# DataArcTech/RAG-ARC

Measured on AMD Instinct MI355X. Metric: queries/sec at fixed (N_corpus, d), exact top-k (ids bit-exact vs CPU oracle), higher is better.
Workload: dtype f16; 1 GPU; 100000000x768 fp16 corpus of N(0,1) directions resident in HBM, row-sharded over 1 GPU(s), batch 256 queries, cosine top-100, exact (canonical fp32 rescore); n_corpus=100000000, d=768, batch=256, k=100, rows_per_gpu=100000000, exchange=none (one shard), repaired_queries_last_step=0

## Files before the change

include/rarc.h:

```cpp
#ifndef RARC_H
#define RARC_H

#include <stddef.h>
#include <stdint.h>

#ifdef __cplusplus
extern "C" {
#endif

#define RARC_VERSION 600

#define RARC_OK 0
#define RARC_E_INVALID -1
#define RARC_E_HIP -2
#define RARC_E_WORKSPACE -3
#define RARC_E_UNSUPPORTED -4
#define RARC_E_IO -5

#define RARC_MAX_QUERIES 256
#define RARC_MAX_K 1024
#define RARC_DIM_ALIGN 128

#define RARC_Q_OK 0u
#define RARC_Q_UNCERTAIN 1u
// ... 261 lines not shown
int rarc_file_to_device(const char* path, int n_seg, const int64_t* h_file_off, const int64_t* h_bytes,
                        const int64_t* h_dev_off, void* d_base, int64_t d_capacity_bytes, void* h_staging,
                        size_t staging_bytes, int n_threads, int flags, void* stream, RarcIoStats* stats);
int rarc_device_to_file(const char* path, int n_seg, const int64_t* h_file_off, const int64_t* h_bytes,
                        const int64_t* h_dev_off, const void* d_base, int64_t d_capacity_bytes, void* h_staging,
                        size_t staging_bytes, int n_threads, int flags, void* stream, RarcIoStats* stats);

size_t rarc_wide_workspace_bytes(int d_pad, int cand_cap);
int rarc_search_wide(const void* d_rows, const uint16_t* d_image16, int fmt, int64_t n_rows, int d_pad, float max_norm,
                     float rho, const void* d_qblock, int nq, int k, int64_t id_base, int64_t* d_out_ids,
                     float* d_out_scores, uint32_t* d_status, void* d_ws, size_t ws_bytes, int cand_cap, void* stream);

int rarc_row_sqnorms(const void* d_rows, int fmt, int64_t n_rows, int d_pad, int64_t first_row, float* d_xn, void* stream);
int rarc_search_wide_l2(const void* d_rows, const uint16_t* d_image16, int fmt, int64_t n_rows, int d_pad, float max_norm,
                        float rho, const float* d_xn, const void* d_qblock, int nq, int k, int64_t id_base, int64_t* d_out_ids,
                        float* d_out_scores, uint32_t* d_status, void* d_ws, size_t ws_bytes, int cand_cap, void* stream);
int rarc_debug_wide_bounds(const void* d_ws, size_t ws_bytes, int d_pad, int cand_cap, float* d_out, void* stream);
int rarc_debug_query_scale8(float mx, float* sq, float* qi);
int rarc_debug_q8_tail_plan(uint32_t t_begin, uint32_t n_tiles, uint32_t grid, int d_pad, int fmt, int pct, int min_mib,
                            uint32_t* t_dyn, uint32_t* r0, uint32_t* unit);
int rarc_debug_q8_tail_chunks(uint32_t k_first, uint32_t n, uint32_t stride, uint32_t unit, uint32_t t_dyn, uint32_t r0,
                              uint32_t n_tiles, uint32_t* t0, uint32_t* t_end);
int64_t rarc_debug_q8_tail_counter_offset(int launch);

size_t rarc_search_rows_workspace_bytes(int nq, int k);
int rarc_search_rows(const void* d_rows, int fmt, int64_t n_rows, int d_pad, const void* d_qblock, int nq, const int64_t* d_list,
                     int64_t m, int k, int64_t id_base, const float* d_xn, int l2, int64_t* d_out_ids, float* d_out_scores,
                     uint32_t* d_status, void* d_ws, size_t ws_bytes, void* stream);
int rarc_strike_rows(const int64_t* d_ids, const float* d_scores, int nq, int kprime, const uint32_t* d_bits, int64_t n_rows,
                     int64_t id_base, int k, int l2, int64_t* d_out_ids, float* d_out_scores, uint32_t* d_count, void* stream);

size_t rarc_search_rows_grouped_workspace_bytes(int nq, int k);
int rarc_search_rows_grouped(const void* d_rows, int fmt, int64_t n_rows, int d_pad, const void* d_qblock, int nq,
                             const int64_t* d_lists, const int64_t* d_tiles, int n_tiles, int64_t m_max, int k, int64_t id_base,
                             const float* d_xn, int l2, int64_t* d_out_ids, float* d_out_scores, uint32_t* d_status, void* d_ws,
                             size_t ws_bytes, void* stream);
int rarc_strike_rows_grouped(const int64_t* d_ids, const float* d_scores, int nq, int kprime, const uint32_t* d_bits,
                             const int64_t* d_bits_off, int64_t n_rows, int64_t id_base, int k, int l2, int64_t* d_out_ids,
                             float* d_out_scores, uint32_t* d_count, void* stream);

size_t rarc_similar_pairs_workspace_bytes(int64_t n_rows, int d, int cand_cap);
int rarc_similar_pairs(const float* d_rows, int64_t ld, int64_t n_rows, int d, double threshold, void* d_ws, size_t ws_bytes,
                       int cand_cap, int64_t* d_out_pairs, double* d_out_scores, int64_t out_cap,
                       unsigned long long* d_out_count, uint32_t* d_flags, void* stream);

size_t rarc_knn_graph_workspace_bytes(int64_t n_rows, int d, int top_k, int cand_cap);
// ... 156 lines not shown
```

rag-arc_amd/csrc/scan_q8.hip:

```cpp
#include "rarc_common.h"
#include <stdio.h>
#ifdef RARC_Q8_ABLATIONS
#include <algorithm>
#endif

struct ScanQ8Params {
  const uint4* corpus;
  const float* tmeta;
  const float* hq;
  const int8_t* q8;
  const float* qinv;
  const float* eps8;
  uint32_t n_rows;
  uint32_t n_tiles;
  uint32_t t_begin;
  uint32_t resume;
  float hot_margin;
  uint32_t* thr;
  const float* binlo;
  const float* binscale;
  const float* bininv;
  uint32_t* hist;
  uint32_t* cnt2;
  uint64_t* cand;
  uint32_t seg;
  uint32_t kprime;
  uint32_t nq;
  uint32_t t_dyn;
  uint32_t tail_r0;
  uint32_t* tail_ctr;
  unsigned long long* dbg;
};

#ifndef Q8_M16_FP16_ROWS
#define Q8_M16_FP16_ROWS 0
#endif
#ifndef Q8_BIG_PF
#define Q8_BIG_PF 1
#endif
#ifndef Q8_BIG_NG
#define Q8_BIG_NG 2
#endif
#ifndef Q8_EB
#define Q8_EB 0
#endif
constexpr int Q8_WAVES = 8;
constexpr int Q8_THREADS = Q8_WAVES * 64;

constexpr int Q8_WSTAGE = 768;
constexpr int Q8_STAGE = 8 * Q8_WSTAGE;
constexpr int Q8_TB_SLOTS = 16;
constexpr int Q8_TB_STRIDE = 80;
constexpr int Q8_DBG_BYTES = 65536;
constexpr int Q8_FIN_SLOT = 2048;
// ... 50 lines not shown
  const uint64_t first = (uint64_t)t_dyn + (uint64_t)start * stride + slot, end = (uint64_t)t_dyn + (uint64_t)(start + r) * stride;
  *t0 = first < n_tiles ? (uint32_t)first : n_tiles;
  *t_end = end < n_tiles ? (uint32_t)end : n_tiles;
}

inline bool q8_tail_plan(uint32_t t_begin, uint32_t n_tiles, uint32_t g, uint32_t unit, uint32_t pct, uint64_t tile_bytes,
                         uint64_t min_bytes, uint32_t* t_dyn, uint32_t* r0) {
  *t_dyn = n_tiles;
  *r0 = 0;
  if (g == 0 || unit == 0 || n_tiles <= t_begin) return false;
  const uint32_t rounds = (uint32_t)(((uint64_t)(n_tiles - t_begin) + g - 1) / g);
  const uint32_t share = (uint32_t)((uint64_t)rounds * (pct > 100u ? 100u : pct) / 100u);
  if (share < unit || (uint64_t)rounds * tile_bytes < min_bytes) return false;
  uint32_t stat = (rounds - share) / unit * unit;
  if (stat < unit) stat = unit;
  const uint64_t td = (uint64_t)t_begin + (uint64_t)stat * g;
  if (td >= n_tiles) return false;
  *t_dyn = (uint32_t)td;
  *r0 = (uint32_t)((((uint64_t)(n_tiles - *t_dyn) + g - 1) / g / 2) / unit * unit);
  return true;
}
inline uint32_t q8_tail_unit(int d_pad) { return d_pad <= 384 ? 4u : 2u; }

template <int D, int FMT = 0, int ABL = 0>
__global__ __launch_bounds__(Q8_THREADS) void rarc_scan_q8_kernel(const ScanQ8Params p) {
  static_assert(D % 128 == 0 && D >= 128 && D <= 1024, "D must be a multiple of 128, <= 1024");
  extern __shared__ __attribute__((aligned(16))) char smem[];
  using L = ScanQ8Lds<D, (FMT != 0) || Q8_M16_FP16_ROWS>;
  constexpr int KS = D / 32;
  static_assert(FMT == 0 || D % 256 == 0, "fp8 rows are padded to a multiple of 256");
  constexpr int EPC = FMT ? 16 : 8;
  constexpr int CPR = D / EPC;
  constexpr int CPT = 32 * CPR / Q8_THREADS;
  constexpr int MSTRIDE = FMT == 1 ? RARC_QMETA_F8_STRIDE : RARC_QMETA_STRIDE;
  constexpr int TCH = 32 * CPR;
  constexpr bool NT_ROWS = !(ABL & 262144);

  const int tid = threadIdx.x;
  const int wave = __builtin_amdgcn_readfirstlane(tid >> 6);
  const int lane = tid & 63;
  const int row = lane & 31, h = lane >> 5;
  constexpr bool M16 = (FMT != 0) || Q8_M16_FP16_ROWS;
  const uint32_t q_lo = wave * 32 + (lane & 15);
  const uint32_t qidx = M16 ? q_lo + 16 * (lane >> 5) : wave * 32 + row;
  const int rq = lane >> 4;
  const int rql = rq & 1;
// ... 23 lines not shown
  if constexpr (M16) {
    const int8_t* qp = p.q8 + (size_t)q_lo * D + 16 * rq;
#pragma unroll
    for (int ks = 0; ks < KS2; ++ks) {
      qf[2 * ks] = *(const i32x4*)(qp + 64 * ks);
      qf[2 * ks + 1] = *(const i32x4*)(qp + 16 * D + 64 * ks);
    }
  } else {
    const int8_t* qp = p.q8 + (size_t)qidx * D + 16 * h;
#pragma unroll
    for (int ks = 0; ks < KS; ++ks) qf[ks] = *(const i32x4*)(qp + 32 * ks);
  }
  const float my_qinv = p.qinv[qidx];
  const float my_hq = p.hq[qidx];
  const float r_max = p.tmeta[0 - RARC_QMETA_HDR];
  float thr = __uint_as_float(p.thr[qidx]);
  __builtin_amdgcn_s_waitcnt(0x0F70);

  constexpr bool WOFF_REGS = (D <= 768);
  auto woff_of = [&](int j) {
    const uint32_t c = j * Q8_THREADS + tid;
    return (c / CPR) * L::RS + (c % CPR) * EPC;
  };
  uint32_t woff[WOFF_REGS ? CPT : 1];
  if constexpr (WOFF_REGS) {
#pragma unroll
    for (int j = 0; j < CPT; ++j) woff[j] = woff_of(j);
  }
  const uint32_t aoff = M16 ? (lane & 15) * L::RS + 16 * rq : row * L::RS + 16 * h;

  const uint32_t stride = gridDim.x;
  uint32_t t0 = p.t_begin + blockIdx.x, t_end = p.tail_ctr ? p.t_dyn : p.n_tiles;
  const bool has_own = blockIdx.x < p.nq;
  const uint32_t own_q = has_own ? blockIdx.x : 0u;
  const uint32_t* hword = p.hist + (size_t)own_q * RARC_NB + 32 * wave + row;

  struct Fetch {
    uint4 c[CPT];
    float mul[FMT == 1 ? CPT : 1];
    float2 meta;
    uint32_t thr;
    uint32_t hw;
  };
  auto clamp_tile = [&](uint32_t t) { return t < t_end ? t : 0u; };
  auto fetch = [&](Fetch& f, uint32_t tile, auto refresh) {
    if constexpr (ABL & 524288) f.meta = make_float2(__uint_as_float(0x7c003c00u), 1.0f);
    else f.meta = *(const float2*)(p.tmeta + (size_t)tile * MSTRIDE);
    if constexpr (FMT == 1) {
#pragma unroll
      for (int j = 0; j < CPT; ++j)
        f.mul[j] = p.tmeta[(size_t)tile * MSTRIDE + 2 + (j * Q8_THREADS + tid) / CPR];
    }
    if constexpr (decltype(refresh)::value) {
      f.thr = __hip_atomic_load(&p.thr[qidx], __ATOMIC_RELAXED, __HIP_MEMORY_SCOPE_AGENT);
      f.hw = __hip_atomic_load(hword, __ATOMIC_RELAXED, __HIP_MEMORY_SCOPE_AGENT);
    }
    __builtin_amdgcn_sched_barrier(0);
    const uint4* src = p.corpus + (size_t)tile * TCH + tid;
#pragma unroll
    for (int j = 0; j < CPT; ++j) {
      if constexpr (NT_ROWS)
        f.c[j] = __builtin_bit_cast(uint4, __builtin_nontemporal_load((const q8_u32x4*)(src + j * Q8_THREADS)));
      else
        f.c[j] = src[j * Q8_THREADS];
    }
  };
  uint32_t opaque_zero = 0;
  asm volatile("" : "+v"(opaque_zero));
  auto convert_chunk = [&](const Fetch& f, int j, half_t s, char* dst) {
    char* at = dst + (WOFF_REGS ? woff[WOFF_REGS ? j : 0] : woff_of(j));
    if constexpr (FMT == 2) {
      const uint4 v = f.c[j];
      *(uint4*)at = make_uint4(v.x ^ opaque_zero, v.y ^ opaque_zero, v.z ^ opaque_zero, v.w ^ opaque_zero);
    } else if constexpr (FMT == 1) {
      if (ABL & 16) {
        const uint4 v = f.c[j];
        *(uint4*)at = make_uint4(v.x ^ opaque_zero, v.y ^ opaque_zero, v.z ^ opaque_zero, v.w ^ opaque_zero);
      } else {
        const uint4 v = rarc_quant8_chunk_f8(f.c[j], (half_t)f.mul[j]);
        if (ABL & 32768) asm volatile("" ::"v"(v.x), "v"(v.y), "v"(v.z), "v"(v.w));
        else *(uint4*)at = v;
      }
    } else {
      uint2 o;
      if (ABL & 16) { o.x = f.c[j].x ^ f.c[j].z; o.y = f.c[j].y ^ f.c[j].w; }
      else o = rarc_quant8_chunk(f.c[j], s);
      *(uint2*)at = o;
    }
  };
  auto convert_tile = [&](const Fetch& f, int buf) {
    const half_t s = q8_tile_scale(f.meta.x);
    char* dst = smem + buf * L::TILE;
#pragma unroll
// ... 10 lines not shown
      constexpr int CSTEP = KS2 / CPT;
      i32x4 a0[PF], a1[PF];
      if (!(ABL & 4) && !((ABL & 65536) && wave >= 4)) {
#pragma unroll
        for (int i = 0; i < PF; ++i) {
          a0[i] = *(const i32x4*)(a_base + 64 * i);
          a1[i] = *(const i32x4*)(a_base + 16 * L::RS + 64 * i);
        }
      }
#pragma unroll
      for (int ks = 0; ks < KS2; ++ks) {
        if (!(ABL & 4) && !((ABL & 65536) && wave >= 4)) {
          c00 = __builtin_amdgcn_mfma_i32_16x16x64_i8(a0[ks % PF], qf[2 * ks], c00, 0, 0, 0);
          c01 = __builtin_amdgcn_mfma_i32_16x16x64_i8(a0[ks % PF], qf[2 * ks + 1], c01, 0, 0, 0);
          c10 = __builtin_amdgcn_mfma_i32_16x16x64_i8(a1[ks % PF], qf[2 * ks], c10, 0, 0, 0);
          c11 = __builtin_amdgcn_mfma_i32_16x16x64_i8(a1[ks % PF], qf[2 * ks + 1], c11, 0, 0, 0);
          if (ks + PF < KS2 && !(ABL & 131072)) {
            a0[ks % PF] = *(const i32x4*)(a_base + 64 * (ks + PF));
            a1[ks % PF] = *(const i32x4*)(a_base + 16 * L::RS + 64 * (ks + PF));
          }
        }
        if (ks % CSTEP == CSTEP / 2) convert_chunk(nx, ks / CSTEP, s, dst);
      }
      if constexpr (D <= 512 || D > 768) RARC_MFMA_SETTLE(c11);
      return (i32x16){c00[0], c00[1], c00[2], c00[3], c10[0], c10[1], c10[2], c10[3],
                      c01[0], c01[1], c01[2], c01[3], c11[0], c11[1], c11[2], c11[3]};
    } else {
      i32x16 c0 = {0};
      constexpr int PF = (D <= 768) ? 4 : 2;
      constexpr int CSTEP = KS / CPT;
      i32x4 a[PF];
      if (!(ABL & 4)) {
#pragma unroll
        for (int i = 0; i < PF; ++i) a[i] = *(const i32x4*)(a_base + 32 * i);
      }
#pragma unroll
      for (int ks = 0; ks < KS; ++ks) {
        if (!(ABL & 4)) {
          c0 = __builtin_amdgcn_mfma_i32_32x32x32_i8(a[ks % PF], qf[ks], c0, 0, 0, 0);
          if (ks + PF < KS) a[ks % PF] = *(const i32x4*)(a_base + 32 * (ks + PF));
        }
        if (ks % CSTEP == CSTEP / 2) convert_chunk(nx, ks / CSTEP, s, dst);
      }
      if constexpr (D <= 512) RARC_MFMA_SETTLE(c0);
      return c0;
    }
  };
  auto regroup = [&](i32x16& a) __attribute__((always_inline)) {
    asm volatile("v_nop\n\tv_nop\n\t"
                 "v_permlane32_swap_b32 %0, %8\n\tv_permlane32_swap_b32 %1, %9\n\tv_permlane32_swap_b32 %2, %10\n\t"
                 "v_permlane32_swap_b32 %3, %11\n\tv_permlane32_swap_b32 %4, %12\n\tv_permlane32_swap_b32 %5, %13\n\t"
                 "v_permlane32_swap_b32 %6, %14\n\tv_permlane32_swap_b32 %7, %15"
                 : "+v"(a[0]), "+v"(a[1]), "+v"(a[2]), "+v"(a[3]), "+v"(a[4]), "+v"(a[5]), "+v"(a[6]), "+v"(a[7]),
                   "+v"(a[8]), "+v"(a[9]), "+v"(a[10]), "+v"(a[11]), "+v"(a[12]), "+v"(a[13]), "+v"(a[14]), "+v"(a[15]));
  };

  auto emit = [&](uint32_t q, uint64_t key, bool hot) {
    const uint32_t slot = atomicAdd(&s_cnt[q], 1u);
    if (slot < p.seg) p.cand[((size_t)q * RARC_MAX_WG + blockIdx.x) * p.seg + slot] = key;
    if (hot) atomicAdd(&p.hist[q * RARC_NB + rarc_bin_of(rarc_candscore(key), s_binlo[q], s_binscale[q])], 1u);
  };
  uint32_t wcount = 0;
  uint64_t* my_skey = s_skey + wave * Q8_WSTAGE;
  uint8_t* my_sq = s_sq + wave * Q8_WSTAGE;
  auto stage_q = [&](bool want, float a, uint32_t doc, uint32_t qq) __attribute__((always_inline)) {
    const unsigned long long b = __builtin_amdgcn_ballot_w64(want);
    if (b == 0) return;
// ... 142 lines not shown
    fetch(f[1], clamp_tile(t0 + stride), Q8Flag<true>{});
    __builtin_amdgcn_sched_barrier(0);
    fetch(f[2], clamp_tile(t0 + 2 * stride), Q8Flag<true>{});
    __builtin_amdgcn_sched_barrier(0);
    fetch(f[3], clamp_tile(t0 + 3 * stride), Q8Flag<true>{});
    __builtin_amdgcn_sched_barrier(0);
    if (!grp_b) fetch(f[0], clamp_tile(t0 + 4 * stride), Q8Flag<true>{});
  } else if constexpr (NG == 2) {
    fetch(f[1], clamp_tile(t0 + stride), Q8Flag<true>{});
    __builtin_amdgcn_sched_barrier(0);
    if (!grp_b) fetch(f[0], clamp_tile(t0 + 2 * stride), Q8Flag<true>{});
  } else {
    fetch(f[0], clamp_tile(t0 + stride), Q8Flag<true>{});
  }
  __builtin_amdgcn_sched_barrier(0);
  __builtin_amdgcn_s_waitcnt(0x0F70);
  q8_lds_barrier();

  i32x16 acc_b = {0};
  bool live_prev = false;
#define Q8_STAMP(slot)                                                                                        \
  if ((ABL & 1024) && blockIdx.x == 0 && it >= 1000 && it < 1016 && lane == 0)                                 \
    p.dbg[8 + ((it - 1000) * Q8_WAVES + wave) * 8 + (slot)] = __builtin_amdgcn_s_memtime();
#define Q8_RF_FETCH(g, par) (!(ABL & 8) && (NG == 1 ? (par) == 1 : (g) == 1))
#define Q8_RF_USE(g, par) (!(ABL & 8) && (NG == 1 ? (par) == 0 : (g) == 1))
#define Q8_ITER(PAR, GB, G, GP)                                                                               \
  {                                                                                                           \
    Q8_STAMP(0)                                                                                               \
    if (!(GB)) {             \
      const float tinv = mcur[PAR].y, tsc = mcur[PAR].x;                                                      \
      i32x16 acc;                                                                                             \
      acc = mfma_convert(PAR, f[G]);                                                                  \
      mcur[(PAR) ^ 1] = f[G].meta;                                                                    \
      Q8_STAMP(1)                                                                                             \
      if (Q8_RF_USE(G, PAR)) {                                                                                \
        thr = fmaxf(thr, __uint_as_float(f[G].thr));                                                  \
        if (lane < 32) s_hland[32 * wave + lane] = f[G].hw;                                           \
      }                                                                                                       \
      if constexpr (EB) {                                \
        Q8_STAMP(3)                                                                                           \
        q8_lds_barrier();                                                                                     \
        Q8_STAMP(4)                                                                                           \
      }                                                                                                       \
      if (!(ABL & 1) && live) prune(acc, cur, tinv, tsc);                                                     \
      else if (q8_all16(acc) == 0x7fffffff) p.cnt2[0] = 1;  \
      Q8_STAMP(2)                                                                                             \
                                                                \
      if (!(ABL & 2)) fetch(f[G], clamp_tile(cur + (NG + 1) * stride), Q8Flag<Q8_RF_FETCH(G, PAR)>{});        \
    } else {  \
      if (!(ABL & 1) && live_prev) prune(acc_b, cur - stride, mcur[(PAR) ^ 1].y, mcur[(PAR) ^ 1].x);          \
      live_prev = live;                                                                                       \
      Q8_STAMP(1)                                                                                             \
      if (!(ABL & 2)) fetch(f[GP], clamp_tile(cur + NG * stride), Q8Flag<Q8_RF_FETCH(GP, PAR)>{});            \
      __builtin_amdgcn_sched_barrier(0);           \
      Q8_STAMP(2)                                                                                             \
      acc_b = mfma_convert(PAR, f[G]);                                                                        \
      mcur[(PAR) ^ 1] = f[G].meta;                                                                            \
      if (Q8_RF_USE(G, PAR)) {                                                                                \
        thr = fmaxf(thr, __uint_as_float(f[G].thr));                                                          \
        if (lane < 32) s_hland[32 * wave + lane] = f[G].hw;                                                   \
      }                                                                                                       \
      if ((ABL & 1) && q8_all16(acc_b) == 0x7fffffff) p.cnt2[0] = 1;                                          \
    }                                                                                                         \
    if constexpr (!EB) {                                                                                      \
      Q8_STAMP(3)                                                                                             \
      q8_lds_barrier();                                                                                       \
      Q8_STAMP(4)                                                                                             \
    }                                                                                                         \
    ++it;                                                                                                     \
                      \
    if (!(ABL & 8) && wave == 0 && has_own && (it <= 16 || (it & 3) == 0)) {                                  \
      const int b = rarc_wave_find_from_top_256(s_hland[4 * lane], s_hland[4 * lane + 1],                     \
                                                s_hland[4 * lane + 2], s_hland[4 * lane + 3], p.kprime);      \
      if (b >= 2 && lane == 0) {                                                                              \
        const float lo = s_binlo[own_q];                                                                      \
        const float t = fmaxf(rarc_bin_threshold(b, lo, s_bininv[own_q]) - 2.0002f * s_eps8[own_q], lo);      \
        if (t > last_pub) {                  \
          last_pub = t;                                                                                       \
          __hip_atomic_store(&p.thr[own_q], __float_as_uint(t), __ATOMIC_RELAXED, __HIP_MEMORY_SCOPE_AGENT);  \
        }                                                                                                     \
      }                                                                                                       \
    }                                                                                                         \
                  \
    if (!(ABL & 64) && (wcount | tb_n) != 0 &&                                                                 \
        (it <= 16 || (it & (it - 1)) == 0 || (it & 127) == 0 || wcount > (uint32_t)Q8_WSTAGE / 2))            \
      flush();                                                                                                \
  }

#define Q8_STEP(OFF, PAR, GB, G, GP)                                                  \
    {                                                                                 \
      const uint32_t cur = base + (OFF) * stride;                                     \
      const bool live = (OFF) == 0 || cur < t_end;                                \
      Q8_ITER(PAR, GB, G, GP)                                                         \
    }
#define Q8_LOOP(GB)                                                                   \
  if constexpr (NG == 4) {                                                            \
    for (uint32_t base = t0; base < t_end; base += 4 * stride) {                  \
      Q8_STEP(0, 0, GB, 1, 0) Q8_STEP(1, 1, GB, 2, 1) Q8_STEP(2, 0, GB, 3, 2) Q8_STEP(3, 1, GB, 0, 3) \
    }                                                                                 \
  } else {                                                                            \
    for (uint32_t base = t0; base < t_end; base += 2 * stride) {                  \
      Q8_STEP(0, 0, GB, NG == 2 ? 1 : 0, 0) Q8_STEP(1, 1, GB, 0, NG == 2 ? 1 : 0)     \
    }                                                                                 \
  }
  if (grp_b) {
    Q8_LOOP(true)
  } else {
    Q8_LOOP(false)
  }
#undef Q8_STEP
#undef Q8_LOOP
#undef Q8_ITER
#undef Q8_RF_FETCH
#undef Q8_RF_USE
  if (grp_b && !(ABL & 1) && live_prev)
    prune(acc_b, t0 + (((t_end - 1 - t0) / stride) | (NG == 4 ? 3u : 1u)) * stride, mcur[1].y, mcur[1].x);
  t0 = p.n_tiles;
  if (p.tail_ctr) {
    uint32_t* s_tick = (uint32_t*)(smem + L::TICK);
    if (tid == 0) *s_tick = atomicAdd(p.tail_ctr, 1u);
    __syncthreads();
    const uint32_t k = __builtin_amdgcn_readfirstlane(*s_tick);
    q8_tail_chunk(k, stride, NG == 4 ? 4u : 2u, p.t_dyn, p.tail_r0, p.n_tiles, &t0, &t_end);
  }
  } while (t0 < p.n_tiles);
  flush();
  __syncthreads();
  if (tid < RARC_MAX_QUERIES) p.cnt2[(size_t)blockIdx.x * RARC_MAX_QUERIES + tid] = s_cnt[tid];
  if (p.dbg && blockIdx.x == 0 && tid == 0) {
    p.dbg[0] = __builtin_amdgcn_s_memtime() - dbg_c0;
    p.dbg[1] = __builtin_amdgcn_s_memrealtime() - dbg_r0;
  }
#ifdef RARC_Q8_ABLATIONS
  if (!(ABL & 1024) && p.dbg && tid == 0) {
// ... 113 lines not shown
        }
        return RARC_OK;
      }
      if (abl == 512) return launch_scan_q8<D, FMT, 512>(p, grid, s);
      if (abl == 17) return launch_scan_q8<D, FMT, 17>(p, grid, s);
      if (abl == 21) return launch_scan_q8<D, FMT, 21>(p, grid, s);
      if (abl == 32769) return launch_scan_q8<D, FMT, 32769>(p, grid, s);
      if (abl == 32773) return launch_scan_q8<D, FMT, 32773>(p, grid, s);
      if (abl == 131073) return launch_scan_q8<D, FMT, 131073>(p, grid, s);
      if (abl == 65536) return launch_scan_q8<D, FMT, 65536>(p, grid, s);
      if (abl == 65537) return launch_scan_q8<D, FMT, 65537>(p, grid, s);
    }
  }
#endif
  hipEvent_t e0, e1;
  const bool prof = rarc_prof_next(&e0, &e1);
  if (prof) RARC_HIP_CHECK(hipEventRecord(e0, s));
  hipLaunchKernelGGL((rarc_scan_q8_kernel<D, FMT, ABL>), dim3(grid), dim3(Q8_THREADS), lds, s, p);
  RARC_HIP_CHECK(hipGetLastError());
  if (prof) RARC_HIP_CHECK(hipEventRecord(e1, s));
  return RARC_OK;
}

template <int FMTV>
static int dispatch_scan_q8(const ScanQ8Params& p, int d_pad, int grid, hipStream_t s) {
  switch (d_pad) {
    case 256: return launch_scan_q8<256, FMTV>(p, grid, s);
    case 512: return launch_scan_q8<512, FMTV>(p, grid, s);
    case 768: return launch_scan_q8<768, FMTV>(p, grid, s);
    case 1024: return launch_scan_q8<1024, FMTV>(p, grid, s);
    default: break;
  }
  if (FMTV == 0) {
    switch (d_pad) {
      case 128: return launch_scan_q8<128, 0>(p, grid, s);
      case 384: return launch_scan_q8<384, 0>(p, grid, s);
      case 640: return launch_scan_q8<640, 0>(p, grid, s);
      case 896: return launch_scan_q8<896, 0>(p, grid, s);
      default: break;
    }
  }
  rarc_set_error("rarc_scan_q8 (row format %d): padded dim %d unsupported (multiple of %d, <= 1024)", FMTV, d_pad,
                 FMTV == 0 ? 128 : 256);
  return RARC_E_UNSUPPORTED;
}

int rarc_scan_q8_launch(const void* corpus, const float* rowscale, int fmt, int64_t n_rows, int d_pad,
                        const float* qmeta, const uint16_t* q16, const int8_t* q8, const float* qinv,
                        const float* eps16, const float* eps8, int nq, int kprime, float bin_lo, float bin_hi,
                        const RarcWs& ws, int cap, int* grid_out, hipStream_t s, const int8_t* shadow8,
                        int (*tighten)(void* ctx, int n_wg, int mode), void* tighten_ctx, const float* hq, const float* floor,
                        int* hybrid_out) {
  ScanQ8Params p;
  p.hq = hq;
  p.corpus = fmt == 2 ? (const uint4*)shadow8 : (const uint4*)corpus;
  p.tmeta = qmeta + RARC_QMETA_HDR;
  p.q8 = q8;
  p.qinv = qinv;
  p.eps8 = eps8;
  p.n_rows = (uint32_t)n_rows;
  p.n_tiles = (uint32_t)((n_rows + 31) / 32);
  p.t_begin = 0;
  p.resume = 0;
  p.hot_margin = 1.0f;
  p.thr = (uint32_t*)ws.thr;
  p.binlo = ws.binlo;
  p.binscale = ws.binscale;
  p.bininv = ws.bininv;
  p.hist = ws.hist;
  p.cnt2 = ws.cnt2;
  p.cand = ws.cand;
  p.seg = (uint32_t)(cap / RARC_MAX_WG);
  p.kprime = (uint32_t)kprime;
  p.nq = (uint32_t)nq;
  p.dbg = nullptr;
  p.t_dyn = p.n_tiles;
  p.tail_r0 = 0;
  p.tail_ctr = nullptr;

  int dev = 0, cus = 256;
  RARC_HIP_CHECK(hipGetDevice(&dev));
  RARC_HIP_CHECK(hipDeviceGetAttribute(&cus, hipDeviceAttributeMultiprocessorCount, dev));
  int grid = cus < RARC_MAX_WG ? cus : RARC_MAX_WG;
  if (const char* e = getenv("RARC_SCAN_Q8_WGS")) { const int g = atoi(e); if (g >= 8 && g < grid) grid = g; }
  if ((uint32_t)grid > p.n_tiles) grid = (int)p.n_tiles;
  *grid_out = grid;
  auto launch = [&](const ScanQ8Params& pp) {
    return fmt == 2 ? dispatch_scan_q8<2>(pp, d_pad, grid, s)
                    : fmt == 1 ? dispatch_scan_q8<1>(pp, d_pad, grid, s) : dispatch_scan_q8<0>(pp, d_pad, grid, s);
  };
  int tail_pct = 16;
  if (const char* e = getenv("RARC_SCAN_Q8_TAIL")) tail_pct = atoi(e);
  tail_pct = tail_pct < 0 ? 0 : (tail_pct > 100 ? 100 : tail_pct);
  int tail_min_mib = 32;
  if (const char* e = getenv("RARC_SCAN_Q8_TAIL_MIN")) tail_min_mib = atoi(e);
  const uint64_t tile_bytes = 32ull * (uint64_t)d_pad * (fmt == 0 ? 2u : 1u);
  static_assert(Q8_DEEP_D == 384, "q8_tail_unit");
  auto set_tail = [&](ScanQ8Params& pp, int launch_idx) {
    const bool tail = q8_tail_plan(pp.t_begin, pp.n_tiles, (uint32_t)grid, q8_tail_unit(d_pad), (uint32_t)tail_pct, tile_bytes,
                                   (uint64_t)(tail_min_mib > 0 ? tail_min_mib : 0) << 20, &pp.t_dyn, &pp.tail_r0);
    pp.tail_ctr = tail ? ws.flags + RARC_WS_TAIL_FLAG + launch_idx : nullptr;
  };
  static const int split_mode = getenv("RARC_SCAN_SPLIT") ? atoi(getenv("RARC_SCAN_SPLIT")) : 3;
  const uint32_t pair = 2u * (uint32_t)(grid > 0 ? grid : 1);
  uint32_t cuts[3];
  int n_cuts = 0;
  if (tighten && split_mode > 0) {
    uint32_t div[3] = {512u, 64u, 8u};
    if (const char* e = getenv("RARC_SPLIT_DIVS")) {
      unsigned a = 0, b = 0, c = 0;
      const int got = sscanf(e, "%u,%u,%u", &a, &b, &c);
      if (got >= 1) { div[0] = a; div[1] = got >= 2 ? b : 0; div[2] = got >= 3 ? c : 0; }
    }
    for (int i = (split_mode >= 3 ? 0 : (split_mode == 2 ? 1 : 2)); i < 3; ++i) {
      if (div[i] == 0) continue;
      const uint32_t t = (p.n_tiles / div[i]) / pair * pair;
      static const int min_env = getenv("RARC_SPLIT_MIN") ? atoi(getenv("RARC_SPLIT_MIN")) : 0;
      const uint32_t min_pairs = min_env > 0 ? (uint32_t)min_env : (div[i] == 8u ? 16u : 8u);
      if (t >= min_pairs * pair && (n_cuts == 0 || t > cuts[n_cuts - 1])) cuts[n_cuts++] = t;
    }
  }
  int rc = rarc_seed_launch(corpus, rowscale, fmt == 2 ? 0 : fmt, n_rows, d_pad, q16, nq, kprime, bin_lo, bin_hi, eps16,
                            eps8, ws, s, n_cuts ? (int64_t)cuts[0] * 32 : 0, floor);
  if (rc) return rc;
  if (p.n_tiles == 0) return RARC_OK;
  RARC_REQUIRE(rarc_gate_scan(s) == 0, RARC_E_HIP, "rarc_scan_q8: hipStreamWaitEvent on the gate event failed");
  uint32_t begin = 0;
  static const int hybrid_env = getenv("RARC_HYBRID") ? atoi(getenv("RARC_HYBRID")) : 1;
  static const int hybrid_div = getenv("RARC_HYBRID_DIV") ? atoi(getenv("RARC_HYBRID_DIV")) : 8;
  if (hybrid_out) *hybrid_out = 0;
  if (hybrid_out && hybrid_env && tighten && fmt == 0 && d_pad <= 768 && n_cuts == 0 && hybrid_div >= 2) {
    const uint32_t stage = (p.n_tiles / (uint32_t)hybrid_div) / pair * pair;
    if (stage >= 2u * pair && stage < p.n_tiles) {
      if ((rc = rarc_scan_f16_stage_launch((const uint16_t*)corpus, n_rows, stage, d_pad, q16, eps16, nq, kprime, ws, cap, grid,
                                           s)) != RARC_OK)
        return rc;
      if ((rc = tighten(tighten_ctx, grid, 2)) != RARC_OK) return rc;
      ScanQ8Params pi = p;
      pi.t_begin = stage;
      pi.resume = 1u;
      pi.hot_margin = 0.f;
      *hybrid_out = 1;
      set_tail(pi, 0);
      return launch(pi);
    }
  }
  for (int i = 0; i <= n_cuts; ++i) {
    ScanQ8Params pi = p;
    pi.t_begin = begin;
    pi.n_tiles = i < n_cuts ? cuts[i] : p.n_tiles;
    pi.resume = i > 0 ? 1u : 0u;
    pi.hot_margin = i > 0 ? 0.f : 1.0f;
    set_tail(pi, i);
    if ((rc = launch(pi)) != RARC_OK) return rc;
    if (i < n_cuts && (rc = tighten(tighten_ctx, grid, 1)) != RARC_OK) return rc;
    begin = pi.n_tiles;
  }
  return RARC_OK;
}

extern "C" int rarc_debug_q8_tail_plan(uint32_t t_begin, uint32_t n_tiles, uint32_t grid, int d_pad, int fmt, int pct, int min_mib,
                                       uint32_t* t_dyn, uint32_t* r0, uint32_t* unit) {
  RARC_REQUIRE(t_dyn && r0 && unit, RARC_E_INVALID, "rarc_debug_q8_tail_plan: null pointer");
  RARC_REQUIRE(d_pad > 0 && fmt >= 0 && fmt <= 2, RARC_E_INVALID, "rarc_debug_q8_tail_plan: d_pad %d, row format %d", d_pad, fmt);
  *unit = q8_tail_unit(d_pad);
  q8_tail_plan(t_begin, n_tiles, grid, *unit, (uint32_t)(pct < 0 ? 0 : pct), 32ull * (uint64_t)d_pad * (fmt == 0 ? 2u : 1u),
               (uint64_t)(min_mib > 0 ? min_mib : 0) << 20, t_dyn, r0);
  return RARC_OK;
}
extern "C" int rarc_debug_q8_tail_chunks(uint32_t k_first, uint32_t n, uint32_t stride, uint32_t unit, uint32_t t_dyn, uint32_t r0,
                                         uint32_t n_tiles, uint32_t* t0, uint32_t* t_end) {
  RARC_REQUIRE(t0 && t_end && stride > 0 && unit > 0, RARC_E_INVALID, "rarc_debug_q8_tail_chunks: null pointer, stride or unit 0");
  for (uint32_t i = 0; i < n; ++i) q8_tail_chunk(k_first + i, stride, unit, t_dyn, r0, n_tiles, &t0[i], &t_end[i]);
  return RARC_OK;
}
extern "C" int64_t rarc_debug_q8_tail_counter_offset(int launch) {
  return launch >= 0 && launch < 4 ? (int64_t)(RARC_WS_FLAGS + 4 * (size_t)(RARC_WS_TAIL_FLAG + launch)) : -1;
}
```

rag-arc_amd/hip/binding.py:

```python
from __future__ import annotations

import ctypes
import os
import threading
from ctypes import c_double, c_float, c_int, c_int64, c_size_t, c_uint64, c_void_p

_PKG = os.path.dirname(os.path.dirname(os.path.abspath(__file__)))
_LIB = os.environ.get("RARC_LIBRARY") or os.path.join(_PKG, "lib", "librarc_hip.so")

MAX_QUERIES = 256
MAX_K = 1024
WIDE_MAX_K = 8192
WIDE_MAX_DPAD = 4096
DIM_ALIGN = 128
Q_UNCERTAIN = 1
Q_OVERFLOW = 2
WS_ANYFLAG_OFFSET = 5124


class RarcError(RuntimeError):
    """Raised for every non-zero status returned by librarc_hip.so."""


class RarcUnsupported(RarcError, NotImplementedError):
# ... 165 lines not shown
    "rarc_lm_gather_last": (c_int, [c_void_p, c_int, c_int, c_int, c_int, c_void_p, c_void_p]),
    "rarc_wordpiece_create": (c_int, [ctypes.c_char_p, c_size_t, c_int, ctypes.c_char_p, ctypes.c_char_p, ctypes.c_char_p,
                                      ctypes.c_char_p, ctypes.c_char_p, c_size_t, c_int, ctypes.POINTER(c_void_p)]),
    "rarc_wordpiece_destroy": (None, [c_void_p]),
    "rarc_wordpiece_encode": (c_int, [c_void_p, ctypes.c_char_p, c_void_p, c_int, c_int, c_void_p, c_int64, c_void_p, c_int]),
    "rarc_file_to_device": (c_int, [ctypes.c_char_p, c_int, ctypes.POINTER(c_int64), ctypes.POINTER(c_int64),
                                    ctypes.POINTER(c_int64), c_void_p, c_int64, c_void_p, c_size_t, c_int, c_int, c_void_p,
                                    ctypes.POINTER(IoStats)]),
    "rarc_device_to_file": (c_int, [ctypes.c_char_p, c_int, ctypes.POINTER(c_int64), ctypes.POINTER(c_int64),
                                    ctypes.POINTER(c_int64), c_void_p, c_int64, c_void_p, c_size_t, c_int, c_int, c_void_p,
                                    ctypes.POINTER(IoStats)]),
    "rarc_wide_workspace_bytes": (c_size_t, [c_int, c_int]),
    "rarc_search_wide": (c_int, [c_void_p, c_void_p, c_int, c_int64, c_int, c_float, c_float, c_void_p, c_int, c_int, c_int64,
                                 c_void_p, c_void_p, c_void_p, c_void_p, c_size_t, c_int, c_void_p]),
    "rarc_row_sqnorms": (c_int, [c_void_p, c_int, c_int64, c_int, c_int64, c_void_p, c_void_p]),
    "rarc_search_wide_l2": (c_int, [c_void_p, c_void_p, c_int, c_int64, c_int, c_float, c_float, c_void_p, c_void_p, c_int, c_int,
                                    c_int64, c_void_p, c_void_p, c_void_p, c_void_p, c_size_t, c_int, c_void_p]),
    "rarc_debug_wide_bounds": (c_int, [c_void_p, c_size_t, c_int, c_int, c_void_p, c_void_p]),
    "rarc_debug_query_scale8": (c_int, [c_float, ctypes.POINTER(c_float), ctypes.POINTER(c_float)]),
    "rarc_debug_q8_tail_plan": (c_int, [ctypes.c_uint32, ctypes.c_uint32, ctypes.c_uint32, c_int, c_int, c_int, c_int,
                                        ctypes.POINTER(ctypes.c_uint32), ctypes.POINTER(ctypes.c_uint32), ctypes.POINTER(ctypes.c_uint32)]),
    "rarc_debug_q8_tail_chunks": (c_int, [ctypes.c_uint32] * 7 + [c_void_p, c_void_p]),
    "rarc_debug_q8_tail_counter_offset": (c_int64, [c_int]),
    "rarc_search_rows_workspace_bytes": (c_size_t, [c_int, c_int]),
    "rarc_search_rows": (c_int, [c_void_p, c_int, c_int64, c_int, c_void_p, c_int, c_void_p, c_int64, c_int, c_int64, c_void_p, c_int,
                                 c_void_p, c_void_p, c_void_p, c_void_p, c_size_t, c_void_p]),
    "rarc_strike_rows": (c_int, [c_void_p, c_void_p, c_int, c_int, c_void_p, c_int64, c_int64, c_int, c_int, c_void_p, c_void_p,
                                 c_void_p, c_void_p]),
    "rarc_search_rows_grouped_workspace_bytes": (c_size_t, [c_int, c_int]),
    "rarc_search_rows_grouped": (c_int, [c_void_p, c_int, c_int64, c_int, c_void_p, c_int, c_void_p, c_void_p, c_int, c_int64, c_int,
                                         c_int64, c_void_p, c_int, c_void_p, c_void_p, c_void_p, c_void_p, c_size_t, c_void_p]),
    "rarc_strike_rows_grouped": (c_int, [c_void_p, c_void_p, c_int, c_int, c_void_p, c_void_p, c_int64, c_int64, c_int, c_int,
                                         c_void_p, c_void_p, c_void_p, c_void_p]),
    "rarc_similar_pairs_workspace_bytes": (c_size_t, [c_int64, c_int, c_int]),
    "rarc_similar_pairs": (c_int, [c_void_p, c_int64, c_int64, c_int, ctypes.c_double, c_void_p, c_size_t, c_int, c_void_p, c_void_p,
                                   c_int64, c_void_p, c_void_p, c_void_p]),
    "rarc_knn_graph_workspace_bytes": (c_size_t, [c_int64, c_int, c_int, c_int]),
    "rarc_knn_graph": (c_int, [c_void_p, c_int64, c_int64, c_int, c_int, ctypes.c_double, c_void_p, c_size_t, c_int, c_void_p, c_void_p,
                               c_void_p, c_void_p, c_void_p]),
    "rarc_graph_csr_workspace_bytes": (c_size_t, [c_int64, c_int64]),
    "rarc_graph_csr": (c_int, [c_void_p, c_void_p, c_void_p, c_int64, c_int64, c_void_p, c_size_t, c_void_p]),
    "rarc_louvain_workspace_bytes": (c_size_t, [c_int64, c_int64]),
    "rarc_louvain_init": (c_int, [c_void_p, c_size_t, c_int64, c_int64, c_void_p, c_size_t, c_void_p, c_void_p]),
    "rarc_louvain_sweep": (c_int, [c_void_p, c_size_t, c_int64, c_int64, c_void_p, c_size_t, c_int, c_int, c_void_p, c_void_p]),
    "rarc_louvain_aggregate": (c_int, [c_void_p, c_size_t, c_int64, c_int64, c_void_p, c_size_t, c_int, c_void_p, c_int64, c_void_p,
                                       c_void_p, c_void_p, c_void_p, c_void_p]),
# ... 131 lines not shown
```

Measured before the change: 9957 queries/s.

## Add settled-pass scan variant refreshing shared threshold only every N tiles

Adds a settled form of the int8 scan kernel that runs on passes after the first, when the threshold is already tightened. In this form the global threshold and histogram refresh (fetch, use, owner lookup) happen once every rf_period loop units instead of every iteration. It also shrinks the per-thread LDS write-offset register array to its repeat period and forces the MFMA settle at D=768. The aim is to cut per-tile synchronisation, global reads and register pressure, at the cost of a staler threshold that may let more candidates through pruning.

```diff
diff --git a/include/rarc.h b/include/rarc.h
--- a/include/rarc.h
+++ b/include/rarc.h
@@ -307,6 +307,9 @@
 int rarc_debug_q8_tail_chunks(uint32_t k_first, uint32_t n, uint32_t stride, uint32_t unit, uint32_t t_dyn, uint32_t r0,
                               uint32_t n_tiles, uint32_t* t0, uint32_t* t_end);
 int64_t rarc_debug_q8_tail_counter_offset(int launch);
+int rarc_debug_q8_refresh_period(int passes_before, uint32_t t_begin, uint32_t t_dyn, uint32_t grid, int d_pad, int fmt, int min_mib,
+                                 int forced, uint32_t* period, uint32_t* default_period);
+int64_t rarc_debug_q8_thr_offset(void);
 
 size_t rarc_search_rows_workspace_bytes(int nq, int k);
 int rarc_search_rows(const void* d_rows, int fmt, int64_t n_rows, int d_pad, const void* d_qblock, int nq, const int64_t* d_list,
diff --git a/rag-arc_amd/csrc/scan_q8.hip b/rag-arc_amd/csrc/scan_q8.hip
--- a/rag-arc_amd/csrc/scan_q8.hip
+++ b/rag-arc_amd/csrc/scan_q8.hip
@@ -30,6 +30,7 @@
   uint32_t tail_r0;
   uint32_t* tail_ctr;
   unsigned long long* dbg;
+  uint32_t rf_period;
 };
 
 #ifndef Q8_M16_FP16_ROWS
@@ -126,6 +127,25 @@
 }
 inline uint32_t q8_tail_unit(int d_pad) { return d_pad <= 384 ? 4u : 2u; }
 
+#ifndef Q8_RF_PERIOD_DEFAULT
+#define Q8_RF_PERIOD_DEFAULT 16
+#endif
+constexpr uint32_t Q8_RF_PERIOD = Q8_RF_PERIOD_DEFAULT;
+constexpr uint64_t Q8_RF_MIN_BYTES = 32ull << 20;
+inline uint32_t q8_refresh_period(int passes_before, uint32_t t_begin, uint32_t t_dyn, uint32_t g, uint64_t tile_bytes,
+                                  uint64_t min_bytes, int forced) {
+  if (forced >= 0) return forced >= 2 ? (uint32_t)forced : 0u;
+  if (passes_before < 1 || g == 0 || t_dyn <= t_begin) return 0u;
+  const uint64_t rounds = ((uint64_t)(t_dyn - t_begin) + g - 1) / g;
+  return rounds * tile_bytes >= min_bytes ? Q8_RF_PERIOD : 0u;
+}
+
+constexpr int Q8_SETTLED = 1048576;
+constexpr int q8_woff_period(int cpr, int cpt) {
+  for (int k = 1; k < cpt; ++k)
+    if ((k * Q8_THREADS) % cpr == 0) return k;
+  return cpt;
+}
 template <int D, int FMT = 0, int ABL = 0>
 __global__ __launch_bounds__(Q8_THREADS) void rarc_scan_q8_kernel(const ScanQ8Params p) {
   static_assert(D % 128 == 0 && D >= 128 && D <= 1024, "D must be a multiple of 128, <= 1024");
@@ -195,10 +215,11 @@
     const uint32_t c = j * Q8_THREADS + tid;
     return (c / CPR) * L::RS + (c % CPR) * EPC;
   };
-  uint32_t woff[WOFF_REGS ? CPT : 1];
+  constexpr int WPER = (ABL & Q8_SETTLED) ? q8_woff_period(CPR, CPT) : CPT;
+  uint32_t woff[WOFF_REGS ? WPER : 1];
   if constexpr (WOFF_REGS) {
 #pragma unroll
-    for (int j = 0; j < CPT; ++j) woff[j] = woff_of(j);
+    for (int j = 0; j < WPER; ++j) woff[j] = woff_of(j);
   }
   const uint32_t aoff = M16 ? (lane & 15) * L::RS + 16 * rq : row * L::RS + 16 * h;
 
@@ -241,7 +262,7 @@
   uint32_t opaque_zero = 0;
   asm volatile("" : "+v"(opaque_zero));
   auto convert_chunk = [&](const Fetch& f, int j, half_t s, char* dst) {
-    char* at = dst + (WOFF_REGS ? woff[WOFF_REGS ? j : 0] : woff_of(j));
+    char* at = dst + (WOFF_REGS ? woff[WOFF_REGS ? j % WPER : 0] + (j / WPER) * (WPER * Q8_THREADS / CPR) * L::RS : woff_of(j));
     if constexpr (FMT == 2) {
       const uint4 v = f.c[j];
       *(uint4*)at = make_uint4(v.x ^ opaque_zero, v.y ^ opaque_zero, v.z ^ opaque_zero, v.w ^ opaque_zero);
@@ -298,7 +319,7 @@
         }
         if (ks % CSTEP == CSTEP / 2) convert_chunk(nx, ks / CSTEP, s, dst);
       }
-      if constexpr (D <= 512 || D > 768) RARC_MFMA_SETTLE(c11);
+      if constexpr (D <= 512 || D > 768 || (ABL & Q8_SETTLED)) RARC_MFMA_SETTLE(c11);
       return (i32x16){c00[0], c00[1], c00[2], c00[3], c10[0], c10[1], c10[2], c10[3],
                       c01[0], c01[1], c01[2], c01[3], c11[0], c11[1], c11[2], c11[3]};
     } else {
@@ -318,7 +339,7 @@
         }
         if (ks % CSTEP == CSTEP / 2) convert_chunk(nx, ks / CSTEP, s, dst);
       }
-      if constexpr (D <= 512) RARC_MFMA_SETTLE(c0);
+      if constexpr (D <= 512 || (ABL & Q8_SETTLED)) RARC_MFMA_SETTLE(c0);
       return c0;
     }
   };
@@ -507,9 +528,10 @@
 #define Q8_STAMP(slot)                                                                                        \
   if ((ABL & 1024) && blockIdx.x == 0 && it >= 1000 && it < 1016 && lane == 0)                                 \
     p.dbg[8 + ((it - 1000) * Q8_WAVES + wave) * 8 + (slot)] = __builtin_amdgcn_s_memtime();
-#define Q8_RF_FETCH(g, par) (!(ABL & 8) && (NG == 1 ? (par) == 1 : (g) == 1))
-#define Q8_RF_USE(g, par) (!(ABL & 8) && (NG == 1 ? (par) == 0 : (g) == 1))
-#define Q8_ITER(PAR, GB, G, GP)                                                                               \
+#define Q8_RF_FETCH(g, par, kind) (!(ABL & 8) && ((kind) == 0 || (kind) == 3) && (NG == 1 ? (par) == 1 : (g) == 1))
+#define Q8_RF_USE(g, par, kind) (!(ABL & 8) && ((kind) == 0 || (kind) == 1) && (NG == 1 ? (par) == 0 : (g) == 1))
+#define Q8_OWNER_LOOK(g, par, kind) ((kind) == 0 ? (it <= 16 || (it & 3) == 0) : Q8_RF_USE(g, par, kind))
+#define Q8_ITER(PAR, GB, G, GP, KIND)                                                                           \
   {                                                                                                           \
     Q8_STAMP(0)                                                                                               \
     if (!(GB)) {             \
@@ -518,7 +540,7 @@
       acc = mfma_convert(PAR, f[G]);                                                                  \
       mcur[(PAR) ^ 1] = f[G].meta;                                                                    \
       Q8_STAMP(1)                                                                                             \
-      if (Q8_RF_USE(G, PAR)) {                                                                                \
+      if (Q8_RF_USE(G, PAR, KIND)) {                                                                                \
         thr = fmaxf(thr, __uint_as_float(f[G].thr));                                                  \
         if (lane < 32) s_hland[32 * wave + lane] = f[G].hw;                                           \
       }                                                                                                       \
@@ -531,17 +553,17 @@
       else if (q8_all16(acc) == 0x7fffffff) p.cnt2[0] = 1;  \
       Q8_STAMP(2)                                                                                             \
                                                                 \
-      if (!(ABL & 2)) fetch(f[G], clamp_tile(cur + (NG + 1) * stride), Q8Flag<Q8_RF_FETCH(G, PAR)>{});        \
+      if (!(ABL & 2)) fetch(f[G], clamp_tile(cur + (NG + 1) * stride), Q8Flag<Q8_RF_FETCH(G, PAR, KIND)>{});  \
     } else {  \
       if (!(ABL & 1) && live_prev) prune(acc_b, cur - stride, mcur[(PAR) ^ 1].y, mcur[(PAR) ^ 1].x);          \
       live_prev = live;                                                                                       \
       Q8_STAMP(1)                                                                                             \
-      if (!(ABL & 2)) fetch(f[GP], clamp_tile(cur + NG * stride), Q8Flag<Q8_RF_FETCH(GP, PAR)>{});            \
+      if (!(ABL & 2)) fetch(f[GP], clamp_tile(cur + NG * stride), Q8Flag<Q8_RF_FETCH(GP, PAR, KIND)>{});      \
       __builtin_amdgcn_sched_barrier(0);           \
       Q8_STAMP(2)                                                                                             \
       acc_b = mfma_convert(PAR, f[G]);                                                                        \
       mcur[(PAR) ^ 1] = f[G].meta;                                                                            \
-      if (Q8_RF_USE(G, PAR)) {                                                                                \
+      if (Q8_RF_USE(G, PAR, KIND)) {                                                                                \
         thr = fmaxf(thr, __uint_as_float(f[G].thr));                                                          \
         if (lane < 32) s_hland[32 * wave + lane] = f[G].hw;                                                   \
       }                                                                                                       \
@@ -554,7 +576,7 @@
     }                                                                                                         \
     ++it;                                                                                                     \
                       \
-    if (!(ABL & 8) && wave == 0 && has_own && (it <= 16 || (it & 3) == 0)) {                                  \
+    if (!(ABL & 8) && wave == 0 && has_own && Q8_OWNER_LOOK(G, PAR, KIND)) {                                  \
       const int b = rarc_wave_find_from_top_256(s_hland[4 * lane], s_hland[4 * lane + 1],                     \
                                                 s_hland[4 * lane + 2], s_hland[4 * lane + 3], p.kprime);      \
       if (b >= 2 && lane == 0) {                                                                              \
@@ -572,29 +594,57 @@
       flush();                                                                                                \
   }
 
-#define Q8_STEP(OFF, PAR, GB, G, GP)                                                  \
+#define Q8_STEP(OFF, PAR, GB, G, GP, KIND)                                            \
     {                                                                                 \
       const uint32_t cur = base + (OFF) * stride;                                     \
       const bool live = (OFF) == 0 || cur < t_end;                                \
-      Q8_ITER(PAR, GB, G, GP)                                                         \
-    }
+      Q8_ITER(PAR, GB, G, GP, KIND)                                                   \
+    }
+#define Q8_UNIT(GB, KIND)                                                             \
+  if constexpr (NG == 4) {                                                            \
+    Q8_STEP(0, 0, GB, 1, 0, KIND) Q8_STEP(1, 1, GB, 2, 1, KIND) Q8_STEP(2, 0, GB, 3, 2, KIND) Q8_STEP(3, 1, GB, 0, 3, KIND) \
+  } else {                                                                            \
+    Q8_STEP(0, 0, GB, NG == 2 ? 1 : 0, 0, KIND) Q8_STEP(1, 1, GB, 0, NG == 2 ? 1 : 0, KIND) \
+  }
 #define Q8_LOOP(GB)                                                                   \
-  if constexpr (NG == 4) {                                                            \
-    for (uint32_t base = t0; base < t_end; base += 4 * stride) {                  \
-      Q8_STEP(0, 0, GB, 1, 0) Q8_STEP(1, 1, GB, 2, 1) Q8_STEP(2, 0, GB, 3, 2) Q8_STEP(3, 1, GB, 0, 3) \
+  for (uint32_t base = t0; base < t_end; base += (NG == 4 ? 4 : 2) * stride) {        \
+    Q8_UNIT(GB, 0)                                                                    \
+  }
+#define Q8_LOOP_SETTLED(GB)                                                           \
+  {                                                                                   \
+    const uint32_t ustep = (NG == 4 ? 4 : 2) * stride;                                \
+    uint32_t base = t0;                                                               \
+    while (base < t_end) {                                                            \
+      Q8_UNIT(GB, 1)                                                                  \
+      base += ustep;                                                                  \
+      if (base >= t_end) break;                                                       \
+      for (uint32_t nq = p.rf_period - 2; nq != 0 && base < t_end; --nq) {            \
+        Q8_UNIT(GB, 2)                                                                \
+        base += ustep;                                                                \
+      }                                                                               \
+      if (base >= t_end) break;                                                       \
+      Q8_UNIT(GB, 3)                                                                  \
+      base += ustep;                                                                  \
     }                                                                                 \
-  } else {                                                                            \
-    for (uint32_t base = t0; base < t_end; base += 2 * stride) {                  \
-      Q8_STEP(0, 0, GB, NG == 2 ? 1 : 0, 0) Q8_STEP(1, 1, GB, 0, NG == 2 ? 1 : 0)     \
-    }                                                                                 \
-  }
-  if (grp_b) {
-    Q8_LOOP(true)
+  }
+  if constexpr (ABL & Q8_SETTLED) {
+    if (grp_b) {
+      Q8_LOOP_SETTLED(true)
+    } else {
+      Q8_LOOP_SETTLED(false)
+    }
   } else {
-    Q8_LOOP(false)
+    if (grp_b) {
+      Q8_LOOP(true)
+    } else {
+      Q8_LOOP(false)
+    }
   }
 #undef Q8_STEP
+#undef Q8_UNIT
 #undef Q8_LOOP
+#undef Q8_LOOP_SETTLED
+#undef Q8_OWNER_LOOK
 #undef Q8_ITER
 #undef Q8_RF_FETCH
 #undef Q8_RF_USE
@@ -754,27 +804,31 @@
   return RARC_OK;
 }
 
-template <int FMTV>
-static int dispatch_scan_q8(const ScanQ8Params& p, int d_pad, int grid, hipStream_t s) {
+template <int FMTV, int FORM>
+static int dispatch_scan_q8_form(const ScanQ8Params& p, int d_pad, int grid, hipStream_t s) {
   switch (d_pad) {
-    case 256: return launch_scan_q8<256, FMTV>(p, grid, s);
-    case 512: return launch_scan_q8<512, FMTV>(p, grid, s);
-    case 768: return launch_scan_q8<768, FMTV>(p, grid, s);
-    case 1024: return launch_scan_q8<1024, FMTV>(p, grid, s);
+    case 256: return launch_scan_q8<256, FMTV, FORM>(p, grid, s);
+    case 512: return launch_scan_q8<512, FMTV, FORM>(p, grid, s);
+    case 768: return launch_scan_q8<768, FMTV, FORM>(p, grid, s);
+    case 1024: return launch_scan_q8<1024, FMTV, FORM>(p, grid, s);
     default: break;
   }
   if (FMTV == 0) {
     switch (d_pad) {
-      case 128: return launch_scan_q8<128, 0>(p, grid, s);
-      case 384: return launch_scan_q8<384, 0>(p, grid, s);
-      case 640: return launch_scan_q8<640, 0>(p, grid, s);
-      case 896: return launch_scan_q8<896, 0>(p, grid, s);
+      case 128: return launch_scan_q8<128, 0, FORM>(p, grid, s);
+      case 384: return launch_scan_q8<384, 0, FORM>(p, grid, s);
+      case 640: return launch_scan_q8<640, 0, FORM>(p, grid, s);
+      case 896: return launch_scan_q8<896, 0, FORM>(p, grid, s);
       default: break;
     }
   }
   rarc_set_error("rarc_scan_q8 (row format %d): padded dim %d unsupported (multiple of %d, <= 1024)", FMTV, d_pad,
                  FMTV == 0 ? 128 : 256);
   return RARC_E_UNSUPPORTED;
+}
+template <int FMTV>
+static int dispatch_scan_q8(const ScanQ8Params& p, int d_pad, int grid, hipStream_t s) {
+  return p.rf_period >= 2 ? dispatch_scan_q8_form<FMTV, Q8_SETTLED>(p, d_pad, grid, s) : dispatch_scan_q8_form<FMTV, 0>(p, d_pad, grid, s);
 }
 
 int rarc_scan_q8_launch(const void* corpus, const float* rowscale, int fmt, int64_t n_rows, int d_pad,
@@ -809,6 +863,7 @@
   p.t_dyn = p.n_tiles;
   p.tail_r0 = 0;
   p.tail_ctr = nullptr;
+  p.rf_period = 0;
 
   int dev = 0, cus = 256;
   RARC_HIP_CHECK(hipGetDevice(&dev));
@@ -828,10 +883,16 @@
   if (const char* e = getenv("RARC_SCAN_Q8_TAIL_MIN")) tail_min_mib = atoi(e);
   const uint64_t tile_bytes = 32ull * (uint64_t)d_pad * (fmt == 0 ? 2u : 1u);
   static_assert(Q8_DEEP_D == 384, "q8_tail_unit");
-  auto set_tail = [&](ScanQ8Params& pp, int launch_idx) {
+  int rf_forced = -1;
+  if (const char* e = getenv("RARC_SCAN_Q8_REFRESH")) { rf_forced = atoi(e); if (rf_forced < 0) rf_forced = 0; }
+  int rf_min_mib = (int)(Q8_RF_MIN_BYTES >> 20);
+  if (const char* e = getenv("RARC_SCAN_Q8_REFRESH_MIN")) rf_min_mib = atoi(e);
+  auto set_tail = [&](ScanQ8Params& pp, int launch_idx, int passes_before) {
     const bool tail = q8_tail_plan(pp.t_begin, pp.n_tiles, (uint32_t)grid, q8_tail_unit(d_pad), (uint32_t)tail_pct, tile_bytes,
                                    (uint64_t)(tail_min_mib > 0 ? tail_min_mib : 0) << 20, &pp.t_dyn, &pp.tail_r0);
     pp.tail_ctr = tail ? ws.flags + RARC_WS_TAIL_FLAG + launch_idx : nullptr;
+    pp.rf_period = q8_refresh_period(passes_before, pp.t_begin, pp.t_dyn, (uint32_t)grid, tile_bytes,
+                                     (uint64_t)(rf_min_mib > 0 ? rf_min_mib : 0) << 20, rf_forced);
   };
   static const int split_mode = getenv("RARC_SCAN_SPLIT") ? atoi(getenv("RARC_SCAN_SPLIT")) : 3;
   const uint32_t pair = 2u * (uint32_t)(grid > 0 ? grid : 1);
@@ -873,7 +934,7 @@
       pi.resume = 1u;
       pi.hot_margin = 0.f;
       *hybrid_out = 1;
-      set_tail(pi, 0);
+      set_tail(pi, 0, 0);
       return launch(pi);
     }
   }
@@ -883,7 +944,7 @@
     pi.n_tiles = i < n_cuts ? cuts[i] : p.n_tiles;
     pi.resume = i > 0 ? 1u : 0u;
     pi.hot_margin = i > 0 ? 0.f : 1.0f;
-    set_tail(pi, i);
+    set_tail(pi, i, i);
     if ((rc = launch(pi)) != RARC_OK) return rc;
     if (i < n_cuts && (rc = tighten(tighten_ctx, grid, 1)) != RARC_OK) return rc;
     begin = pi.n_tiles;
@@ -906,6 +967,16 @@
   for (uint32_t i = 0; i < n; ++i) q8_tail_chunk(k_first + i, stride, unit, t_dyn, r0, n_tiles, &t0[i], &t_end[i]);
   return RARC_OK;
 }
+extern "C" int rarc_debug_q8_refresh_period(int passes_before, uint32_t t_begin, uint32_t t_dyn, uint32_t grid, int d_pad, int fmt,
+                                            int min_mib, int forced, uint32_t* period, uint32_t* default_period) {
+  RARC_REQUIRE(period && default_period, RARC_E_INVALID, "rarc_debug_q8_refresh_period: null pointer");
+  RARC_REQUIRE(d_pad > 0 && fmt >= 0 && fmt <= 2, RARC_E_INVALID, "rarc_debug_q8_refresh_period: d_pad %d, row format %d", d_pad, fmt);
+  *period = q8_refresh_period(passes_before, t_begin, t_dyn, grid, 32ull * (uint64_t)d_pad * (fmt == 0 ? 2u : 1u),
+                              min_mib < 0 ? Q8_RF_MIN_BYTES : (uint64_t)min_mib << 20, forced);
+  *default_period = Q8_RF_PERIOD;
+  return RARC_OK;
+}
+extern "C" int64_t rarc_debug_q8_thr_offset(void) { return (int64_t)RARC_WS_THR; }
 extern "C" int64_t rarc_debug_q8_tail_counter_offset(int launch) {
   return launch >= 0 && launch < 4 ? (int64_t)(RARC_WS_FLAGS + 4 * (size_t)(RARC_WS_TAIL_FLAG + launch)) : -1;
 }
diff --git a/rag-arc_amd/hip/binding.py b/rag-arc_amd/hip/binding.py
--- a/rag-arc_amd/hip/binding.py
+++ b/rag-arc_amd/hip/binding.py
@@ -211,6 +211,9 @@
                                         ctypes.POINTER(ctypes.c_uint32), ctypes.POINTER(ctypes.c_uint32), ctypes.POINTER(ctypes.c_uint32)]),
     "rarc_debug_q8_tail_chunks": (c_int, [ctypes.c_uint32] * 7 + [c_void_p, c_void_p]),
     "rarc_debug_q8_tail_counter_offset": (c_int64, [c_int]),
+    "rarc_debug_q8_thr_offset": (c_int64, []),
+    "rarc_debug_q8_refresh_period": (c_int, [c_int, ctypes.c_uint32, ctypes.c_uint32, ctypes.c_uint32, c_int, c_int, c_int, c_int,
+                                             ctypes.POINTER(ctypes.c_uint32), ctypes.POINTER(ctypes.c_uint32)]),
     "rarc_search_rows_workspace_bytes": (c_size_t, [c_int, c_int]),
     "rarc_search_rows": (c_int, [c_void_p, c_int, c_int64, c_int, c_void_p, c_int, c_void_p, c_int64, c_int, c_int64, c_void_p, c_int,
                                  c_void_p, c_void_p, c_void_p, c_void_p, c_size_t, c_void_p]),
```

After: 10110 queries/s (median of 6 runs). 1.01x the previous value.
